# NeRF-3DTalker/NeRF-3DTalker-code

Measured on AMD Instinct MI355X. Metric: rendered frames/sec @512^2 x 64 samples/ray, higher is better.
Workload: dtype bf16; 1 GPU; cfg2-R: 16 heads/GPU/step, 64x64 rays x 64 samples -> fused MLP+composite -> neural renderer -> 512x512 RGB (+ background image); rays_per_frame=4096, samples_per_ray=64, parallelism=frames sharded over 1 rank(s), no data-path collective, ranks_seen_by_backend=1

## Files before the change

nerf-3dtalker-code_amd/csrc/nerf_aux.hip:

```cpp
#include "n3dt_device.h"
#include "n3dt_layout.h"
#include "n3dt_launch.h"

__device__ __forceinline__ float logical_weight(const N3dtMlpParams& p, int stage, int row, int col, int S, int A, int U) {
    const int in0 = N3DT_PE_DIM + S + U, in5 = N3DT_PE_DIM + S + N3DT_HID, inr = N3DT_HID + A;
    switch (stage) {
        case 0: return col < N3DT_PE_DIM ? p.weight[0][(size_t)row * in0 + col] : 0.0f;
        case 5:
            if (col < N3DT_PE_DIM) return p.weight[5][(size_t)row * in5 + col];
            if (col == N3DT_PE_DIM) return 0.0f;
            return p.weight[5][(size_t)row * in5 + N3DT_PE_DIM + S + (col - 64)];
        case 8: return row == 0 ? p.weight[8][col] : 0.0f;
        case 10: return p.weight[10][(size_t)row * inr + col];
        default: return p.weight[stage][(size_t)row * N3DT_HID + col];
    }
}

__global__ __launch_bounds__(256) void small_gemm_kernel(int M, int N, int K, const float* __restrict__ A, long sam, long sak,
                                                                 const float* __restrict__ Bm, long sbn, long sbk,
                                                                 float* __restrict__ C, long ldc, int accumulate) {
    __shared__ float As[32][33], Bs[32][33];
    const int t = threadIdx.x, tx = t & 15, ty = t >> 4;
    const int m0 = blockIdx.y * 32, n0 = blockIdx.x * 32;
    float acc[2][2] = {{0.f, 0.f}, {0.f, 0.f}};
// ... 190 lines not shown
    }
}

extern "C" void n3dt_launch_fold(const N3dtGeom* g, const N3dtMlpParams* p, const float* shape, const float* appea,
                                 const float* audio, float* fold, int merged_rgb, hipStream_t stream) {
    hipLaunchKernelGGL(fold_latents_kernel, dim3(g->batch, N3DT_NSTAGE, FOLD_ROWGROUPS), dim3(256), 0, stream, *p, g->shape_dim,
                       g->appea_dim, g->audio_dim, merged_rgb, shape, appea, audio, fold);
}

__global__ __launch_bounds__(256) void rayfold_kernel(int n_rays, long total, const float* __restrict__ fold, const float* __restrict__ ray_bias,
                                                      float* __restrict__ rayfold) {
    const long i = (long)blockIdx.x * blockDim.x + threadIdx.x;
    if (i >= total * 48) return;
    const long ray = i / 48;
    const int o = (int)(i % 48) * 4;
    const f32x4 f = *reinterpret_cast<const f32x4*>(fold + (size_t)(ray / n_rays) * N3DT_FOLD_STRIDE + n3dt_bias_offset(10) + o);
    const f32x4 r = *reinterpret_cast<const f32x4*>(ray_bias + (size_t)ray * N3DT_RAYFOLD_STRIDE + o);
    *reinterpret_cast<f32x4*>(rayfold + (size_t)ray * N3DT_RAYFOLD_STRIDE + o) = f32x4{f[0] + r[0], f[1] + r[1], f[2] + r[2], f[3] + r[3]};
}
extern "C" void n3dt_launch_rayfold(const N3dtGeom* g, const float* fold, const float* ray_bias, hipStream_t s) {
    const long total = (long)g->batch * g->n_rays;
    float* rayfold = const_cast<float*>(fold) + n3dt_rayfold_offset(g->batch);
    hipLaunchKernelGGL(rayfold_kernel, dim3((unsigned)((total * 48 + 255) / 256)), dim3(256), 0, s, g->n_rays, total, fold, ray_bias, rayfold);
}

__global__ __launch_bounds__(256) void ray_vd_bias_kernel(N3dtGeom g, const float* __restrict__ w_vd, long ld_w, const float* __restrict__ xy,
                                                          const float* __restrict__ R, const float* __restrict__ Kinv,
                                                          float* __restrict__ ray_bias) {
    __shared__ float wl[192 * 27];
    for (int i = threadIdx.x; i < 192 * 27; i += blockDim.x) wl[i] = w_vd[(size_t)(i / 27) * ld_w + i % 27];
    __syncthreads();
    const int lane = threadIdx.x & 63, wave = threadIdx.x >> 6;
    const long total = (long)g.batch * g.n_rays;
    for (long rayg = (long)blockIdx.x * 4 + wave; rayg < total; rayg += (long)gridDim.x * 4) {
        const int b = (int)(rayg / g.n_rays), ray = (int)(rayg % g.n_rays);
        const float x = xy[(int64_t)b * g.xy_stride_b + 0 * g.xy_stride_c + (int64_t)ray * g.xy_stride_r];
        const float y = xy[(int64_t)b * g.xy_stride_b + 1 * g.xy_stride_c + (int64_t)ray * g.xy_stride_r];
        float d[3], l;
        n3dt_ray_setup(R + b * 9, Kinv + b * 9, x, y, d, l);
        float pe[27];
        pe[0] = d[0]; pe[1] = d[1]; pe[2] = d[2];
#pragma unroll
        for (int k = 0; k < 4; ++k)
#pragma unroll
            for (int i = 0; i < 3; ++i) {
                const float a = d[i] * (float)(1 << k);
                pe[3 + 6 * k + i] = sinf(a);
                pe[3 + 6 * k + 3 + i] = cosf(a);
            }
#pragma unroll
        for (int u = 0; u < 3; ++u) {
            const int o = lane + 64 * u;
            float acc = 0.0f;
#pragma unroll
            for (int j = 0; j < 27; ++j) acc = fmaf(wl[o * 27 + j], pe[j], acc);
            ray_bias[(size_t)rayg * N3DT_RAYFOLD_STRIDE + o] = acc;
        }
    }
}
extern "C" void n3dt_launch_ray_vd_bias(const N3dtGeom* g, const float* w_vd, long ld_w, const float* xy, const float* R, const float* Kinv,
                                        float* ray_bias, hipStream_t s) {
    const long total = (long)g->batch * g->n_rays;
    long grid = (total + 3) / 4;
    if (grid > 2048) grid = 2048;
    hipLaunchKernelGGL(ray_vd_bias_kernel, dim3((unsigned)grid), dim3(256), 0, s, *g, w_vd, ld_w, xy, R, Kinv, ray_bias);
}

#define HEAD_RAYS 8
#define HEAD_MAX_BPR 64
__global__ __launch_bounds__(256) void ray_head_kernel(N3dtGeom g, int bpr, int bs, const float* __restrict__ part,
                                                       const float* __restrict__ wlocal, const float* __restrict__ tail,
                                                       const float* __restrict__ bg_featmap, int bg_hwc, float* __restrict__ fg_feat,
                                                       float* __restrict__ bg_alpha, float* __restrict__ depth,
                                                       float* __restrict__ weight, float* __restrict__ merge_feat,
                                                       float* __restrict__ rayrec) {
    __shared__ float G[HEAD_RAYS][N3DT_G];
    __shared__ float pref[HEAD_RAYS][HEAD_MAX_BPR];
    __shared__ float wsum_s[HEAD_RAYS], dsum_s[HEAD_RAYS];
    const long nrays_total = (long)g.batch * g.n_rays;
    const long ray0 = (long)blockIdx.x * HEAD_RAYS;
    const int t = threadIdx.x;
    if (t < HEAD_RAYS) {
        long rg = ray0 + t;
        float Trun = 1.0f, ws = 0.0f, ds = 0.0f;
        if (rg < nrays_total) {
            for (int k = 0; k < bpr; ++k) {
                const float* po = part + ((size_t)rg * bpr + k) * N3DT_PART_STRIDE + N3DT_G;
                pref[t][k] = Trun;
                ws += Trun * po[0];
                ds += Trun * po[1];
                Trun *= po[2];
            }
        }
        wsum_s[t] = ws;
        dsum_s[t] = ds;
    }
    __syncthreads();
    for (int i = t; i < HEAD_RAYS * N3DT_G; i += 256) {
        int r = i / N3DT_G, j = i % N3DT_G;
        long rg = ray0 + r;
        float acc = 0.0f;
        if (rg < nrays_total)
            for (int k = 0; k < bpr; ++k) acc += pref[r][k] * part[((size_t)rg * bpr + k) * N3DT_PART_STRIDE + j];
        G[r][j] = acc;
        if (rayrec && rg < nrays_total) rayrec[(size_t)rg * N3DT_PART_STRIDE + j] = acc;
    }
    __syncthreads();
    if (rayrec && t < HEAD_RAYS && ray0 + t < nrays_total) {
        float* rec = rayrec + (size_t)(ray0 + t) * N3DT_PART_STRIDE + N3DT_G;
        rec[0] = wsum_s[t];
        rec[1] = dsum_s[t];
        rec[2] = 0.0f;
        rec[3] = 0.0f;
    }
    const float* W2T = tail;
    const float b2 = tail[N3DT_G * N3DT_C + t];
    float acc[HEAD_RAYS];
#pragma unroll
    for (int r = 0; r < HEAD_RAYS; ++r) acc[r] = 0.0f;
    for (int j = 0; j < N3DT_G; ++j) {
        float wv = W2T[j * N3DT_C + t];
#pragma unroll
        for (int r = 0; r < HEAD_RAYS; ++r) acc[r] = fmaf(wv, G[r][j], acc[r]);
    }
#pragma unroll
    for (int r = 0; r < HEAD_RAYS; ++r) {
        long rg = ray0 + r;
        if (rg >= nrays_total) break;
        float fg = acc[r] + b2 * wsum_s[r];
        float ba = 1.0f - wsum_s[r];
        if (fg_feat) fg_feat[(size_t)rg * N3DT_C + t] = fg;
        if (merge_feat) {
            int ray = (int)(rg % g.n_rays);
            merge_feat[(size_t)rg * N3DT_C + t] = fg + ba * (bg_hwc ? bg_featmap[(size_t)ray * N3DT_C + t] : bg_featmap[(size_t)t * g.n_rays + ray]);
        }
        if (t == 0) {
            if (bg_alpha) bg_alpha[rg] = ba;
            if (depth) depth[rg] = dsum_s[r];
        }
    }
    if (weight) {
        for (int i = t; i < HEAD_RAYS * g.n_samples; i += 256) {
            int r = i / g.n_samples, s = i % g.n_samples;
            long rg = ray0 + r;
            if (rg < nrays_total) {
                int k = s / bs;
                weight[(size_t)rg * g.n_samples + s] = pref[r][k] * wlocal[((size_t)rg * bpr + k) * bs + (s % bs)];
            }
        }
    }
}

typedef __bf16 rh_bf16x8 __attribute__((ext_vector_type(8)));
#define RH_RAYS 32
template <bool MAP16, int PREC16 = N3DT_BF16>
__global__ __launch_bounds__(256, 4) void ray_head_mfma_kernel(N3dtGeom g, int bpr, int bs, const float* __restrict__ part,
                                                            const float* __restrict__ wlocal, const float* __restrict__ tail,
                                                            const float* __restrict__ bg_featmap, int bg_hwc,
                                                            float* __restrict__ fg_feat, float* __restrict__ bg_alpha,
                                                            float* __restrict__ depth, float* __restrict__ weight,
                                                            float* __restrict__ merge_feat, float* __restrict__ rayrec,
                                                            unsigned short* __restrict__ merge16, float* __restrict__ rgb0, const float* __restrict__ rgb_w,
                                                            const float* __restrict__ rgb_b) {
    __shared__ __attribute__((aligned(16))) float G[RH_RAYS][N3DT_G + 4];
    __shared__ float pref[RH_RAYS][HEAD_MAX_BPR];
    __shared__ float wsum_s[RH_RAYS], dsum_s[RH_RAYS];
    __shared__ float rgb_s[4][RH_RAYS][3];
    const long nrays_total = (long)g.batch * g.n_rays;
    const long ray0 = (long)blockIdx.x * RH_RAYS;
    const int t = threadIdx.x, lane = t & 63, wave = t >> 6;
    if (MAP16) rayrec = nullptr;
    if (t < RH_RAYS) {
        const long rg = ray0 + t;
        float Trun = 1.0f, ws = 0.0f, ds = 0.0f;
        if (rg < nrays_total) {
            for (int k = 0; k < bpr; ++k) {
                const float* po = part + ((size_t)rg * bpr + k) * N3DT_PART_STRIDE + N3DT_G;
                pref[t][k] = Trun;
                ws += Trun * po[0];
                ds += Trun * po[1];
                Trun *= po[2];
            }
        }
        wsum_s[t] = ws;
        dsum_s[t] = ds;
    }
    __syncthreads();
    static_assert(N3DT_G % 4 == 0 && (N3DT_PART_STRIDE * 4) % 16 == 0 && RH_RAYS * (N3DT_G / 4) % 256 == 0, "whole quads");
    constexpr int QPR = N3DT_G / 4, NQ = RH_RAYS * QPR / 256;
    if (bpr <= 2) {
        f32x4 v[NQ][2];
        float pf[NQ][2];
#pragma unroll
        for (int u = 0; u < NQ; ++u) {
            const int i = t + 256 * u, r = i / QPR, q = i % QPR;
            const long rg = min(ray0 + r, nrays_total - 1);
            const float* p0 = part + (size_t)rg * bpr * N3DT_PART_STRIDE + 4 * q;
            v[u][0] = *reinterpret_cast<const f32x4*>(p0);
            v[u][1] = *reinterpret_cast<const f32x4*>(p0 + (bpr == 2 ? N3DT_PART_STRIDE : 0));
            pf[u][0] = pref[r][0];
            pf[u][1] = bpr == 2 ? pref[r][1] : 0.0f;
        }
#pragma unroll
        for (int u = 0; u < NQ; ++u) {
            const int i = t + 256 * u, r = i / QPR, q = i % QPR;
            f32x4 a;
#pragma unroll
            for (int e = 0; e < 4; ++e) a[e] = pf[u][0] * v[u][0][e] + pf[u][1] * v[u][1][e];
            const bool in = ray0 + r < nrays_total;
            if (!in) a = f32x4{0.0f, 0.0f, 0.0f, 0.0f};
            *reinterpret_cast<f32x4*>(&G[r][4 * q]) = a;
            if (rayrec && in) *reinterpret_cast<f32x4*>(rayrec + (size_t)(ray0 + r) * N3DT_PART_STRIDE + 4 * q) = a;
        }
    } else {
        for (int i = t; i < RH_RAYS * N3DT_G; i += 256) {
            const int r = i / N3DT_G, j = i % N3DT_G;
            const long rg = ray0 + r;
            float acc = 0.0f;
            if (rg < nrays_total)
                for (int k = 0; k < bpr; ++k) acc += pref[r][k] * part[((size_t)rg * bpr + k) * N3DT_PART_STRIDE + j];
            G[r][j] = acc;
            if (rayrec && rg < nrays_total) rayrec[(size_t)rg * N3DT_PART_STRIDE + j] = acc;
        }
    }
    __syncthreads();
    if (rayrec && t < RH_RAYS && ray0 + t < nrays_total) {
        float* rec = rayrec + (size_t)(ray0 + t) * N3DT_PART_STRIDE + N3DT_G;
        rec[0] = wsum_s[t];
        rec[1] = dsum_s[t];
        rec[2] = 0.0f;
        rec[3] = 0.0f;
    }
    const int r31 = lane & 31, h = lane >> 5;
    f32x16 acc[2];
#pragma unroll
    for (int i = 0; i < 2; ++i)
#pragma unroll
        for (int r = 0; r < 16; ++r) acc[i][r] = 0.0f;
    const rh_bf16x8* w2frags = reinterpret_cast<const rh_bf16x8*>(tail + n3dt_tail_w2_frags_offset());
#pragma unroll 2
    for (int ks = 0; ks < N3DT_G / 16; ++ks) {
        const int k0 = 16 * ks + 8 * h;
        rh_bf16x8 a_hi, a_lo;
        const f32x4 g0 = *reinterpret_cast<const f32x4*>(&G[r31][k0]), g1 = *reinterpret_cast<const f32x4*>(&G[r31][k0 + 4]);
#pragma unroll
        for (int j = 0; j < 8; ++j) {
            const float v = j < 4 ? g0[j] : g1[j - 4];
            const __bf16 hi = (__bf16)v;
            a_hi[j] = hi;
            a_lo[j] = (__bf16)(v - (float)hi);
        }
#pragma unroll
        for (int i = 0; i < 2; ++i) {
            const rh_bf16x8* fr = w2frags + ((size_t)(ks * 8 + 2 * wave + i) * 2) * 64 + lane;
            const rh_bf16x8 b_hi = fr[0], b_lo = fr[64];
            acc[i] = __builtin_amdgcn_mfma_f32_32x32x16_bf16(a_hi, b_hi, acc[i], 0, 0, 0);
            acc[i] = __builtin_amdgcn_mfma_f32_32x32x16_bf16(a_hi, b_lo, acc[i], 0, 0, 0);
            acc[i] = __builtin_amdgcn_mfma_f32_32x32x16_bf16(a_lo, b_hi, acc[i], 0, 0, 0);
        }
    }
    float pr[MAP16 ? 16 : 1][3];
    if constexpr (!MAP16) {
#pragma unroll
        for (int i = 0; i < 2; ++i) {
            const int c = 64 * wave + 32 * i + r31;
            const float b2 = tail[N3DT_G * N3DT_C + c];
            float bgv[16];
#pragma unroll
            for (int r = 0; r < 16; ++r) {
                const int rr = (r & 3) + 8 * (r >> 2) + 4 * h;
                const long rg = min(ray0 + rr, nrays_total - 1);
                const int ray = (int)(rg % g.n_rays);
                bgv[r] = merge_feat ? (bg_hwc ? bg_featmap[(size_t)ray * N3DT_C + c] : bg_featmap[(size_t)c * g.n_rays + ray]) : 0.0f;
            }
#pragma unroll
            for (int r = 0; r < 16; ++r) {
                const int rr = (r & 3) + 8 * (r >> 2) + 4 * h;
                const long rg = ray0 + rr;
                if (rg >= nrays_total) continue;
                const float fg = acc[i][r] + b2 * wsum_s[rr];
                if (fg_feat) fg_feat[(size_t)rg * N3DT_C + c] = fg;
                if (merge_feat) merge_feat[(size_t)rg * N3DT_C + c] = fg + (1.0f - wsum_s[rr]) * bgv[r];
            }
        }
    } else {
#pragma unroll
        for (int i = 0; i < 2; ++i) {
            const int c = 64 * wave + 32 * i + r31;
            const float b2 = tail[N3DT_G * N3DT_C + c];
            float w3[3] = {0.0f, 0.0f, 0.0f};
            if (rgb0) {
#pragma unroll
                for (int k = 0; k < 3; ++k) w3[k] = rgb_w[k * N3DT_C + c];
            }
#pragma unroll
            for (int r0 = 0; r0 < 16; r0 += 8) {
                float bgv[8];
#pragma unroll
                for (int r = r0; r < r0 + 8; ++r) {
                    const int rr = (r & 3) + 8 * (r >> 2) + 4 * h;
                    const long rg = min(ray0 + rr, nrays_total - 1);
                    const int ray = (int)(rg % g.n_rays);
                    bgv[r - r0] = bg_featmap[(size_t)ray * N3DT_C + c];
                }
#pragma unroll
                for (int r = r0; r < r0 + 8; ++r) {
                    const int rr = (r & 3) + 8 * (r >> 2) + 4 * h;
                    const long rg = ray0 + rr;
                    const float mg = (acc[i][r] + b2 * wsum_s[rr]) + (1.0f - wsum_s[rr]) * bgv[r - r0];
#pragma unroll
                    for (int k = 0; k < 3; ++k) pr[MAP16 ? r : 0][k] = i == 0 ? w3[k] * mg : fmaf(w3[k], mg, pr[MAP16 ? r : 0][k]);
                    if (merge16 && rg < nrays_total)
                        merge16[(size_t)rg * N3DT_C + c] = PREC16 == N3DT_BF16 ? __builtin_bit_cast(unsigned short, (__bf16)mg)
                                                                               : __builtin_bit_cast(unsigned short, (_Float16)mg);
                }
                __builtin_amdgcn_sched_barrier(0);
            }
            __builtin_amdgcn_sched_barrier(0);
        }
    }
    if constexpr (MAP16) if (rgb0) {
#pragma unroll
        for (int step = 0; step < 4; ++step) {
            const int n = 8 >> step, off = 16 >> step;
            const bool up = (r31 & off) != 0;
#pragma unroll
            for (int r = 0; r < n; ++r)
#pragma unroll
                for (int k = 0; k < 3; ++k) {
                    const float keep = up ? pr[r + n][k] : pr[r][k], send = up ? pr[r][k] : pr[r + n][k];
                    pr[r][k] = keep + __shfl_xor(send, off, 64);
                }
        }
#pragma unroll
        for (int k = 0; k < 3; ++k) pr[0][k] += __shfl_xor(pr[0][k], 1, 64);
        if ((r31 & 1) == 0) {
            const int rsel = (r31 >> 1) & 15;
            const int rr = (rsel & 3) + 8 * (rsel >> 2) + 4 * h;
#pragma unroll
            for (int k = 0; k < 3; ++k) rgb_s[wave][rr][k] = pr[0][k];
        }
        __syncthreads();
        if (t < 3 * RH_RAYS) {
            const int rr = t % RH_RAYS, k = t / RH_RAYS;
            const long rg = ray0 + rr;
            if (rg < nrays_total) {
                const float v = (rgb_s[0][rr][k] + rgb_s[1][rr][k]) + (rgb_s[2][rr][k] + rgb_s[3][rr][k]) + rgb_b[k];
                const long img = rg / g.n_rays, p = rg % g.n_rays;
                rgb0[(size_t)(img * 3 + k) * g.n_rays + p] = v;
            }
        }
    }
    if (t < RH_RAYS && ray0 + t < nrays_total) {
        if (bg_alpha) bg_alpha[ray0 + t] = 1.0f - wsum_s[t];
        if (depth) depth[ray0 + t] = dsum_s[t];
    }
    if (weight) {
        for (int i = t; i < RH_RAYS * g.n_samples; i += 256) {
            const int r = i / g.n_samples, s = i % g.n_samples;
            const long rg = ray0 + r;
            if (rg < nrays_total) {
                const int k = s / bs;
                weight[(size_t)rg * g.n_samples + s] = pref[r][k] * wlocal[((size_t)rg * bpr + k) * bs + (s % bs)];
            }
        }
    }
}

extern "C" void n3dt_launch_ray_head_mfma(const N3dtGeom* g, int bpr, int bs, const float* part, const float* wlocal,
                                          const float* tail, const float* bg_featmap, int bg_hwc, float* fg_feat, float* bg_alpha,
                                          float* depth, float* weight, float* merge_feat, float* rayrec, hipStream_t stream) {
    const long nrays_total = (long)g->batch * g->n_rays;
    const int grid = (int)((nrays_total + RH_RAYS - 1) / RH_RAYS);
    hipLaunchKernelGGL(ray_head_mfma_kernel<false>, dim3(grid), dim3(256), 0, stream, *g, bpr, bs, part, wlocal, tail,
                       merge_feat ? bg_featmap : nullptr, bg_hwc, fg_feat, bg_alpha, depth, weight, merge_feat, rayrec,
                       (unsigned short*)nullptr, (float*)nullptr, (const float*)nullptr, (const float*)nullptr);
}

extern "C" void n3dt_launch_ray_head_mfma16(const N3dtGeom* g, int bpr, int bs, const float* part, const float* wlocal,
                                            const float* tail, const float* bg_featmap, int bg_hwc, float* fg_feat, float* bg_alpha,
                                            float* depth, float* weight, float* merge_feat, void* merge16, int prec16, float* rgb0,
                                            const float* rgb_w, const float* rgb_b, hipStream_t stream) {
    const long nrays_total = (long)g->batch * g->n_rays;
    const int grid = (int)((nrays_total + RH_RAYS - 1) / RH_RAYS);
    if (fg_feat || merge_feat) {
        hipLaunchKernelGGL(ray_head_mfma_kernel<false>, dim3(grid), dim3(256), 0, stream, *g, bpr, bs, part, wlocal, tail,
                           merge_feat ? bg_featmap : nullptr, bg_hwc, fg_feat, (float*)nullptr, (float*)nullptr, (float*)nullptr, merge_feat,
                           (float*)nullptr, (unsigned short*)nullptr, (float*)nullptr, (const float*)nullptr, (const float*)nullptr);
    }
    if (prec16 == N3DT_BF16)
        hipLaunchKernelGGL((ray_head_mfma_kernel<true, N3DT_BF16>), dim3(grid), dim3(256), 0, stream, *g, bpr, bs, part, wlocal, tail, bg_featmap,
                           bg_hwc, (float*)nullptr, bg_alpha, depth, weight, (float*)nullptr, (float*)nullptr,
                           reinterpret_cast<unsigned short*>(merge16), rgb0, rgb_w, rgb_b);
    else
        hipLaunchKernelGGL((ray_head_mfma_kernel<true, N3DT_F16>), dim3(grid), dim3(256), 0, stream, *g, bpr, bs, part, wlocal, tail, bg_featmap,
                           bg_hwc, (float*)nullptr, bg_alpha, depth, weight, (float*)nullptr, (float*)nullptr,
                           reinterpret_cast<unsigned short*>(merge16), rgb0, rgb_w, rgb_b);
}

extern "C" void n3dt_launch_ray_head(const N3dtGeom* g, int bpr, int bs, const float* part, const float* wlocal,
                                     const float* tail, const float* bg_featmap, int bg_hwc, float* fg_feat, float* bg_alpha,
                                     float* depth, float* weight, float* merge_feat, hipStream_t stream) {
    const long nrays_total = (long)g->batch * g->n_rays;
    const int grid = (int)((nrays_total + HEAD_RAYS - 1) / HEAD_RAYS);
    hipLaunchKernelGGL(ray_head_kernel, dim3(grid), dim3(256), 0, stream, *g, bpr, bs, part, wlocal, tail,
                       merge_feat ? bg_featmap : nullptr, bg_hwc, fg_feat, bg_alpha, depth, weight, merge_feat, (float*)nullptr);
}

// ... 127 lines not shown
```

nerf-3dtalker-code_amd/csrc/nr_blur_mfma.inc:

```
#define NBM_TR 4
#define NBM_TC 8
#define NBM_IMG 4096
#define NBM_BUF (NBM_IMG + 512)
#define NBM_WAVE (2 * NBM_BUF)

template <int N>
__device__ __forceinline__ void nbm_wait_vm() {
    asm volatile("s_waitcnt vmcnt(%0)" ::"i"(N) : "memory");
}

template <int PREC, bool NET>
__global__ __launch_bounds__(256) void blur_mfma_q_kernel(const int nb, const int H, const int W, const int K, const unsigned short* __restrict__ hid,
                                                          const float* __restrict__ bias, unsigned short* __restrict__ net,
                                                          const float* __restrict__ Wrgb, const float* __restrict__ brgb,
                                                          const float* __restrict__ rgb_lo, float* __restrict__ rgb_out, const int final_sigmoid,
                                                          float* __restrict__ rgb_out2, const int n_tiles) {
    typedef typename X16<PREC>::frag frag;
    extern __shared__ __attribute__((aligned(16))) unsigned char lds[];
    const int wave = __builtin_amdgcn_readfirstlane(threadIdx.x >> 6);
    const int lane = threadIdx.x & 63, c = lane & 31, hh = lane >> 5;
    const int nchunk = K >> 5;
    unsigned char* const wave_lds = lds + wave * NBM_WAVE;
    unsigned char* const a2_lds = lds + 4 * NBM_WAVE;
    float* const bias_lds = reinterpret_cast<float*>(a2_lds + (size_t)nchunk * 2 * 2 * 2 * 3 * 16);
// ... 136 lines not shown
    nimg = img; nR0 = R0; nC0 = C0;
    setup_tile(img, R0, C0);
    issue_item(0, 0);
    int younger = 0;
    float p0 = 0.0f, p1 = 0.0f;
    f32x16 acc2;
    for (;;) {
        const int R = R0 + (c >> 3), C = C0 + (c & 7);
        int nt = t, nc = chunk + 1;
        if (nc == nchunk) {
            nt = t + nw;
            nc = 0;
        }
        const bool has_next = nt < n_tiles;
        if (younger >= 5) nbm_wait_vm<5>();
        else if (younger >= 3) nbm_wait_vm<3>();
        else if (younger >= 2) nbm_wait_vm<2>();
        else nbm_wait_vm<0>();
        const unsigned img_addr = wave_addr + buf * NBM_BUF + tr_off;
        x16_u32x2 q0[4], q1[4];
        x16_tr_issue<0>(q0[0], img_addr);
        x16_tr_issue<256>(q1[0], img_addr);
        x16_tr_issue<1024>(q0[1], img_addr);
        x16_tr_issue<1280>(q1[1], img_addr);
        x16_tr_issue<2048>(q0[2], img_addr);
        x16_tr_issue<2304>(q1[2], img_addr);
        x16_tr_issue<3072>(q0[3], img_addr);
        x16_tr_issue<3328>(q1[3], img_addr);
        if (chunk == 0) {
#pragma unroll
            for (int r = 0; r < 16; ++r) acc2[r] = 0.0f;
            p0 = p1 = 0.0f;
            if (rgb_lo) {
                const float* win = reinterpret_cast<const float*>(wave_lds + buf * NBM_BUF + NBM_IMG) + ((R >> 1) - (R0 >> 1)) * 6 + ((C >> 1) - (C0 >> 1));
                float wr[3] = {wr_in[0], wr_in[1], wr_in[2]}, wc[3] = {wc_in[0], wc_in[1], wc_in[2]};
                if (R0 < 2 || R0 + NBM_TR > H2 - 2 || H < 3) n3dt_up_blur_w3(R, H, wr);
                if (C0 < 2 || C0 + NBM_TC > W2 - 2 || W < 3) n3dt_up_blur_w3(C, W, wc);
                const float* wa = win + (hh ? 48 : 0);
                float tmp[3] = {0.0f, 0.0f, 0.0f}, tm1[3] = {0.0f, 0.0f, 0.0f};
#pragma unroll
                for (int a = 0; a < 3; ++a)
#pragma unroll
                    for (int b = 0; b < 3; ++b) {
                        tmp[b] = fmaf(wr[a], wa[6 * a + b], tmp[b]);
                        tm1[b] = fmaf(wr[a], win[24 + 6 * a + b], tm1[b]);
                    }
#pragma unroll
                for (int b = 0; b < 3; ++b) {
                    p0 = fmaf(wc[b], tmp[b], p0);
                    p1 = fmaf(wc[b], tm1[b], p1);
                }
            }
        }
        const f32x4* bp = reinterpret_cast<const f32x4*>(bias_lds + chunk * 32 + hh * 16);
        const f32x4 bq0 = bp[0], bq1 = bp[1], bq2 = bp[2], bq3 = bp[3];
        x16_tr_settle();
#pragma unroll
        for (int s = 0; s < 4; ++s) asm volatile("" : "+v"(q0[s]), "+v"(q1[s]));
        if (has_next) {
            if (nc == 0) {
                where(nt, nimg, nR0, nC0);
                setup_tile(nimg, nR0, nC0);
            }
            issue_item(nc, buf ^ 1);
        }
        younger = 0;
        f32x16 acc;
#pragma unroll
        for (int r = 0; r < 16; ++r) acc[r] = 0.0f;
#pragma unroll
        for (int s = 0; s < 4; ++s) {
            const x16_u32x4 v = {q0[s][0], q0[s][1], q1[s][0], q1[s][1]};
            acc = X16<PREC>::mfma(__builtin_bit_cast(frag, v), S[s], acc);
        }
        const float bb[16] = {bq0[0], bq0[1], bq0[2], bq0[3], bq1[0], bq1[1], bq1[2], bq1[3],
                              bq2[0], bq2[1], bq2[2], bq2[3], bq3[0], bq3[1], bq3[2], bq3[3]};
        float v[16];
#pragma unroll
        for (int r = 0; r < 16; ++r) {
            const float a = fmaf(acc[r], 0.0625f, bb[r]);
            v[r] = fmaxf(a, 0.2f * a);
        }
        const frag f0 = X16<PREC>::pack(v), f1 = X16<PREC>::pack(v + 8);
        if (NET) {
            unsigned char* const tb = wave_lds + buf * NBM_BUF;
            const x16_u32x4 w0 = __builtin_bit_cast(x16_u32x4, f0), w1 = __builtin_bit_cast(x16_u32x4, f1);
            unsigned char* const wrow = tb + c * 72 + 8 * hh;
            *reinterpret_cast<x16_u32x2*>(wrow) = x16_u32x2{w0[0], w0[1]};
            *reinterpret_cast<x16_u32x2*>(wrow + 16) = x16_u32x2{w0[2], w0[3]};
            *reinterpret_cast<x16_u32x2*>(wrow + 32) = x16_u32x2{w1[0], w1[1]};
            *reinterpret_cast<x16_u32x2*>(wrow + 48) = x16_u32x2{w1[2], w1[3]};
            __builtin_amdgcn_fence(__ATOMIC_RELEASE, "wavefront");
            __builtin_amdgcn_wave_barrier();
            __builtin_amdgcn_fence(__ATOMIC_ACQUIRE, "wavefront");
            unsigned char* const nbase = reinterpret_cast<unsigned char*>(net) + ((((size_t)img * H2 + R0) * W2 + C0) * K + chunk * 32) * 2;
#pragma unroll
            for (int jj = 0; jj < 2; ++jj) {
                const unsigned char* rrow = tb + ((lane >> 2) + 16 * jj) * 72 + 16 * (lane & 3);
                const x16_u32x2 lo = *reinterpret_cast<const x16_u32x2*>(rrow), hi = *reinterpret_cast<const x16_u32x2*>(rrow + 8);
                *reinterpret_cast<x16_u32x4*>(nbase + soff[jj]) = x16_u32x4{lo[0], lo[1], hi[0], hi[1]};
            }
            younger += 2;
        }
        {
            const unsigned char* ap = a2_lds + (size_t)(((chunk * 2) * 2 * 2 + hh) * 3 + (c < 3 ? c : 0)) * 16;
            const frag z = __builtin_bit_cast(frag, x16_u32x4{0u, 0u, 0u, 0u});
            const frag t0h = *reinterpret_cast<const frag*>(ap), t0l = *reinterpret_cast<const frag*>(ap + 6 * 16);
            const frag t1h = *reinterpret_cast<const frag*>(ap + 12 * 16), t1l = *reinterpret_cast<const frag*>(ap + 18 * 16);
            const bool live = c < 3;
            acc2 = X16<PREC>::mfma(live ? t0l : z, f0, acc2);
            acc2 = X16<PREC>::mfma(live ? t1l : z, f1, acc2);
            acc2 = X16<PREC>::mfma(live ? t0h : z, f0, acc2);
            acc2 = X16<PREC>::mfma(live ? t1h : z, f1, acc2);
        }
        if (nc == 0) {
            const float p2 = __shfl(p0, c + 32, 64);
            if (!hh) {
                float r0 = acc2[0] + b0 + p0, r1 = acc2[1] + b1 + p1, r2 = acc2[2] + b2 + p2;
                if (final_sigmoid) {
                    r0 = 1.0f / (1.0f + __expf(-r0));
                    r1 = 1.0f / (1.0f + __expf(-r1));
                    r2 = 1.0f / (1.0f + __expf(-r2));
                }
                const size_t o = (size_t)img * 3 * HW2 + (size_t)R * W2 + C;
                rgb_out[o] = r0;
                rgb_out[o + HW2] = r1;
                rgb_out[o + 2 * HW2] = r2;
                if (rgb_out2) {
                    rgb_out2[o] = r0;
                    rgb_out2[o + HW2] = r1;
                    rgb_out2[o + 2 * HW2] = r2;
                }
            }
            younger += 3;
        }
        if (!has_next) break;
        t = nt;
        chunk = nc;
        buf ^= 1;
        img = nimg;
        R0 = nR0;
        C0 = nC0;
    }
}

#define NBM8_SLOTS 112
#define NBM8_IMG (NBM8_SLOTS * 64)
#define NBM8_BUF (NBM8_IMG + 512)
#ifndef NBM8_DB
#define NBM8_DB 0
#endif
#define NBM8_WAVE ((NBM8_DB ? 2 : 1) * NBM8_BUF)

template <int PREC>
__global__ __launch_bounds__(256) void blur_mfma_last_kernel(const int nb, const int H, const int W, const unsigned short* __restrict__ hid,
                                                             const float* __restrict__ bias, const float* __restrict__ Wrgb,
                                                             const float* __restrict__ brgb, const float* __restrict__ rgb_lo,
                                                             float* __restrict__ rgb_out, const int final_sigmoid, float* __restrict__ rgb_out2,
                                                             const int n_tiles) {
    typedef typename X16<PREC>::frag frag;
    constexpr int K = 32;
    extern __shared__ __attribute__((aligned(16))) unsigned char lds[];
    const int wave = __builtin_amdgcn_readfirstlane(threadIdx.x >> 6);
    const int lane = threadIdx.x & 63, c = lane & 31, hh = lane >> 5;
    unsigned char* const wave_lds = lds + wave * NBM8_WAVE;
    unsigned char* const a2_lds = lds + 4 * NBM8_WAVE;
    float* const bias_lds = reinterpret_cast<float*>(a2_lds + 2 * 2 * 2 * 3 * 16);

    for (int i = threadIdx.x; i < 2 * 2 * 3; i += blockDim.x) {
        const int row = i % 3, half = (i / 3) & 1, s = i / 6;
        float w[8], rem[8];
#pragma unroll
        for (int e = 0; e < 8; ++e) {
            const int r = 8 * s + e, ch = (r & 3) + 8 * (r >> 2) + 4 * half;
            w[e] = Wrgb[(size_t)row * K + ch];
        }
        const frag hi = X16<PREC>::pack(w);
#pragma unroll
        for (int e = 0; e < 8; ++e) rem[e] = w[e] - (float)hi[e];
        const frag lo = X16<PREC>::pack(rem);
        *reinterpret_cast<frag*>(a2_lds + (size_t)((((s * 2 + 0) * 2 + half) * 3 + row) * 16)) = hi;
        *reinterpret_cast<frag*>(a2_lds + (size_t)((((s * 2 + 1) * 2 + half) * 3 + row) * 16)) = lo;
    }
    for (int i = threadIdx.x; i < 32; i += blockDim.x) {
        const int half = i >> 4, r = i & 15;
        bias_lds[i] = bias[(r & 3) + 8 * (r >> 2) + 4 * half];
    }
    asm volatile("s_waitcnt vmcnt(0)" ::: "memory");
    __syncthreads();

    frag S[4];
    {
        const int orow = c >> 3, ocol = c & 7;
#pragma unroll
        for (int s = 0; s < 4; ++s) {
            float w[8];
#pragma unroll
            for (int e = 0; e < 8; ++e) {
                const int k = 16 * s + 8 * hh + e, hr = k / 10, hc = k - 10 * hr;
                const int dr = hr - orow, dc = hc - ocol;
                const float wr = (k < 60 && dr >= 0 && dr <= 2) ? (dr == 1 ? 2.0f : 1.0f) : 0.0f;
                const float wc = (dc >= 0 && dc <= 2) ? (dc == 1 ? 2.0f : 1.0f) : 0.0f;
                w[e] = wr * wc;
            }
            S[s] = X16<PREC>::pack(w);
        }
    }
    const bool live = c < 3;
    const frag z = __builtin_bit_cast(frag, x16_u32x4{0u, 0u, 0u, 0u});
    frag t0h, t0l, t1h, t1l;
    {
        const unsigned char* ap = a2_lds + (size_t)((hh * 3 + (live ? c : 0)) * 16);
        t0h = *reinterpret_cast<const frag*>(ap);
        t0l = *reinterpret_cast<const frag*>(ap + 6 * 16);
        t1h = *reinterpret_cast<const frag*>(ap + 12 * 16);
        t1l = *reinterpret_cast<const frag*>(ap + 18 * 16);
        if (!live) t0h = t0l = t1h = t1l = z;
    }
    const int H2 = 2 * H, W2 = 2 * W;
    const size_t Mq = (size_t)nb * H * W;
    int ioff[7];
#pragma unroll
    for (int i = 0; i < 7; ++i) {
        int k = 16 * i + (lane >> 2);
        if (k > 99) k = 99;
        const int hr = k / 10, hc = k - 10 * hr;
        const int q = 2 * ((hr + 1) & 1) + ((hc + 1) & 1);
        const long dR = (hr - 1) >> 1, dC = (hc - 1) >> 1;
        ioff[i] = (int)((((long)q * (long)Mq + dR * W + dC) * K + 8 * (lane & 3)) * 2);
    }
    int pch[2], prow[2], pcol[2];
#pragma unroll
    for (int i = 0; i < 2; ++i) {
        int j = 64 * i + lane;
        if (j > 107) j = 107;
        pch[i] = j / 36;
        prow[i] = (j - 36 * pch[i]) / 6;
        pcol[i] = j - 36 * pch[i] - 6 * prow[i];
    }
    const unsigned img_addr = (unsigned)(size_t)(LDS_AS unsigned char*)wave_lds + x16_tr_lane_offset_natural(lane);
    const int tiles_x = W2 / 8, tiles_y = H2 / 8, per_img = tiles_x * tiles_y;
    const int tx_shift = (tiles_x & (tiles_x - 1)) == 0 ? 31 - __builtin_clz(tiles_x) : -1;
    const int ty_shift = (tiles_y & (tiles_y - 1)) == 0 ? 31 - __builtin_clz(tiles_y) : -1;
    const bool pow2 = tx_shift >= 0 && ty_shift >= 0;
    auto where = [&](const int t, int& img, int& R0, int& C0) {
        if (pow2) {
            C0 = (t & (tiles_x - 1)) * 8;
            R0 = ((t >> tx_shift) & (tiles_y - 1)) * 8;
            img = t >> (tx_shift + ty_shift);
        } else {
            img = t / per_img;
            const int tt = t - img * per_img, ty = tt / tiles_x;
            R0 = ty * 8;
            C0 = (tt - ty * tiles_x) * 8;
        }
    };
    const bool r_ev = ((c >> 3) & 1) == 0, c_ev = (c & 1) == 0;
    const float wr_in[3] = {r_ev ? 0.3125f : 0.0625f, 0.625f, r_ev ? 0.0625f : 0.3125f};
    const float wc_in[3] = {c_ev ? 0.3125f : 0.0625f, 0.625f, c_ev ? 0.0625f : 0.3125f};
    const size_t HW2 = (size_t)H2 * W2;
    const float b0 = brgb[0], b1 = brgb[1], b2 = brgb[2];
    const int nw = gridDim.x * 4;

    auto issue_item = [&](const int img, const int R0, const int C0, const int buf) {
        unsigned char* const dstb = wave_lds + buf * NBM8_BUF;
        if (rgb_lo) {
#pragma unroll
            for (int i = 0; i < 2; ++i) {
                const int hr = min(max((R0 >> 1) - 1 + prow[i], 0), H - 1), wc = min(max((C0 >> 1) - 1 + pcol[i], 0), W - 1);
                const float* ps = rgb_lo + (((size_t)img * 3 + pch[i]) * H + hr) * W + wc;
                __builtin_amdgcn_global_load_lds((const GLOBAL_AS void*)ps, (LDS_AS void*)(dstb + NBM8_IMG + 256 * i), 4, 0, 0);
            }
        }
        const bool interior = R0 > 0 && R0 + 8 < H2 && C0 > 0 && C0 + 8 < W2;
        if (interior) {
            const unsigned char* base = reinterpret_cast<const unsigned char*>(hid) + (((size_t)img * H + (R0 >> 1)) * W + (C0 >> 1)) * K * 2;
#pragma unroll
            for (int i = 0; i < 7; ++i)
                __builtin_amdgcn_global_load_lds((const GLOBAL_AS void*)(base + ioff[i]), (LDS_AS void*)(dstb + i * 1024), 16, 0, 0);
        } else {
#pragma unroll
            for (int i = 0; i < 7; ++i) {
                int k = 16 * i + (lane >> 2);
                if (k > 99) k = 99;
                const int hr = k / 10, hc = k - 10 * hr;
                const int R = hreflect1(R0 - 1 + hr, H2), C = hreflect1(C0 - 1 + hc, W2);
                const int q = 2 * (R & 1) + (C & 1);
                const unsigned char* sp = reinterpret_cast<const unsigned char*>(hid) +
                                          (((size_t)q * Mq + ((size_t)img * H + (R >> 1)) * W + (C >> 1)) * K + 8 * (lane & 3)) * 2;
                __builtin_amdgcn_global_load_lds((const GLOBAL_AS void*)sp, (LDS_AS void*)(dstb + i * 1024), 16, 0, 0);
            }
        }
    };

    int t = blockIdx.x * 4 + wave;
    if (t >= n_tiles) return;
    int img, R0, C0;
    where(t, img, R0, C0);
    issue_item(img, R0, C0, 0);
    bool first = true;
    int buf = 0;
    for (;;) {
        const int nt = t + nw;
        const bool has_next = nt < n_tiles;
        if (first) nbm_wait_vm<0>();
        else nbm_wait_vm<NBM8_DB ? 6 : 3>();
        first = false;
        int nimg = img, nR0 = R0, nC0 = C0;
        if (NBM8_DB && has_next) {
            where(nt, nimg, nR0, nC0);
            issue_item(nimg, nR0, nC0, buf ^ 1);
        }
        const unsigned cur_addr = img_addr + buf * NBM8_BUF;
        float p0[2] = {0.0f, 0.0f}, p1[2] = {0.0f, 0.0f};
        if (rgb_lo) {
            const float* win0 = reinterpret_cast<const float*>(wave_lds + buf * NBM8_BUF + NBM8_IMG);
            const bool edge_c = C0 == 0 || C0 + 8 == W2 || W < 3;
#pragma unroll
            for (int j = 0; j < 2; ++j) {
                const int R = R0 + 4 * j + (c >> 3), C = C0 + (c & 7);
                float wr[3] = {wr_in[0], wr_in[1], wr_in[2]}, wc[3] = {wc_in[0], wc_in[1], wc_in[2]};
                if ((j == 0 && R0 == 0) || (j == 1 && R0 + 8 == H2) || H < 3) n3dt_up_blur_w3(R, H, wr);
                if (edge_c) n3dt_up_blur_w3(C, W, wc);
                const float* win = win0 + ((R >> 1) - (R0 >> 1)) * 6 + ((C >> 1) - (C0 >> 1));
                const float* wa = win + (hh ? 72 : 0);
                float tmp[3] = {0.0f, 0.0f, 0.0f}, tm1[3] = {0.0f, 0.0f, 0.0f};
#pragma unroll
                for (int a = 0; a < 3; ++a)
#pragma unroll
                    for (int b = 0; b < 3; ++b) {
                        tmp[b] = fmaf(wr[a], wa[6 * a + b], tmp[b]);
                        tm1[b] = fmaf(wr[a], win[36 + 6 * a + b], tm1[b]);
                    }
#pragma unroll
                for (int b = 0; b < 3; ++b) {
                    p0[j] = fmaf(wc[b], tmp[b], p0[j]);
                    p1[j] = fmaf(wc[b], tm1[b], p1[j]);
                }
            }
        }
#pragma unroll
        for (int j = 0; j < 2; ++j) {
            x16_u32x2 q0[4], q1[4];
            if (j == 0) {
                x16_tr_issue<0>(q0[0], cur_addr);
                x16_tr_issue<256>(q1[0], cur_addr);
                x16_tr_issue<1024>(q0[1], cur_addr);
                x16_tr_issue<1280>(q1[1], cur_addr);
                x16_tr_issue<2048>(q0[2], cur_addr);
                x16_tr_issue<2304>(q1[2], cur_addr);
                x16_tr_issue<3072>(q0[3], cur_addr);
                x16_tr_issue<3328>(q1[3], cur_addr);
            } else {
                x16_tr_issue<2560 + 0>(q0[0], cur_addr);
                x16_tr_issue<2560 + 256>(q1[0], cur_addr);
                x16_tr_issue<2560 + 1024>(q0[1], cur_addr);
                x16_tr_issue<2560 + 1280>(q1[1], cur_addr);
                x16_tr_issue<2560 + 2048>(q0[2], cur_addr);
                x16_tr_issue<2560 + 2304>(q1[2], cur_addr);
                x16_tr_issue<2560 + 3072>(q0[3], cur_addr);
                x16_tr_issue<2560 + 3328>(q1[3], cur_addr);
            }
            x16_tr_settle();
#pragma unroll
            for (int s = 0; s < 4; ++s) asm volatile("" : "+v"(q0[s]), "+v"(q1[s]));
            if (!NBM8_DB && j == 1 && has_next) {
                where(nt, nimg, nR0, nC0);
                issue_item(nimg, nR0, nC0, 0);
            }
            f32x16 acc;
#pragma unroll
            for (int r = 0; r < 16; ++r) acc[r] = 0.0f;
#pragma unroll
            for (int s = 0; s < 4; ++s) {
                const x16_u32x4 v = {q0[s][0], q0[s][1], q1[s][0], q1[s][1]};
                acc = X16<PREC>::mfma(__builtin_bit_cast(frag, v), S[s], acc);
            }
            float v[16];
            {
                const f32x4* bp = reinterpret_cast<const f32x4*>(bias_lds + hh * 16);
                const f32x4 bq0 = bp[0], bq1 = bp[1], bq2 = bp[2], bq3 = bp[3];
                const float bb[16] = {bq0[0], bq0[1], bq0[2], bq0[3], bq1[0], bq1[1], bq1[2], bq1[3],
                                      bq2[0], bq2[1], bq2[2], bq2[3], bq3[0], bq3[1], bq3[2], bq3[3]};
#pragma unroll
                for (int r = 0; r < 16; ++r) {
                    const float a = fmaf(acc[r], 0.0625f, bb[r]);
                    v[r] = fmaxf(a, 0.2f * a);
                }
            }
            const frag f0 = X16<PREC>::pack(v), f1 = X16<PREC>::pack(v + 8);
            f32x16 acc2;
#pragma unroll
            for (int r = 0; r < 16; ++r) acc2[r] = 0.0f;
            acc2 = X16<PREC>::mfma(t0l, f0, acc2);
            acc2 = X16<PREC>::mfma(t1l, f1, acc2);
            acc2 = X16<PREC>::mfma(t0h, f0, acc2);
            acc2 = X16<PREC>::mfma(t1h, f1, acc2);
            const float p2 = __shfl(p0[j], c + 32, 64);
            if (!hh) {
                const int R = R0 + 4 * j + (c >> 3), C = C0 + (c & 7);
                float r0 = acc2[0] + b0 + p0[j], r1 = acc2[1] + b1 + p1[j], r2 = acc2[2] + b2 + p2;
                if (final_sigmoid) {
                    r0 = 1.0f / (1.0f + __expf(-r0));
                    r1 = 1.0f / (1.0f + __expf(-r1));
                    r2 = 1.0f / (1.0f + __expf(-r2));
                }
                const size_t o = (size_t)img * 3 * HW2 + (size_t)R * W2 + C;
                rgb_out[o] = r0;
                rgb_out[o + HW2] = r1;
                rgb_out[o + 2 * HW2] = r2;
                if (rgb_out2) {
                    rgb_out2[o] = r0;
                    rgb_out2[o + HW2] = r1;
                    rgb_out2[o + 2 * HW2] = r2;
                }
            }
        }
        if (!has_next) break;
        t = nt;
        img = nimg;
        R0 = nR0;
        C0 = nC0;
        if (NBM8_DB) buf ^= 1;
    }
}

static inline bool nbm_supported(int nb, int H, int W, int K) {
    const char* e = getenv("N3DT_NR_BLUR_MFMA");
    if (e && atoi(e) == 0) return false;
    if (H < 2 || W < 4 || (H & 1) || (W & 3) || (K & 31) || K > 256) return false;
    return (size_t)4 * nb * H * W * K * 2 < ((size_t)1 << 31);
}

template <int PREC>
static void launch_blur_q(int nb, int H, int W, int K, const unsigned short* hid, const float* bias, unsigned short* net, const float* Wrgb,
                          const float* brgb, const float* rgb_lo, float* rgb_out, int final_sigmoid, float* rgb_out2, hipStream_t s) {
    if (!net && K == 32 && !(H & 3) && nbm_supported(nb, H, W, K) && !(getenv("N3DT_NR_BLUR_TILE8") && atoi(getenv("N3DT_NR_BLUR_TILE8")) == 0)) {
        const int n_tiles = nb * (2 * H / 8) * (2 * W / 8);
        const size_t lds_bytes = 4 * NBM8_WAVE + 2 * 2 * 2 * 3 * 16 + 32 * sizeof(float);
        auto kern = blur_mfma_last_kernel<PREC>;
        static int cus8 = 0, occ8 = 0;
        if (cus8 == 0) {
            int dev = 0, n = 0;
            (void)hipGetDevice(&dev);
            (void)hipDeviceGetAttribute(&n, hipDeviceAttributeMultiprocessorCount, dev);
            cus8 = n > 0 ? n : 256;
        }
        if (occ8 == 0 && (hipOccupancyMaxActiveBlocksPerMultiprocessor(&occ8, reinterpret_cast<const void*>(kern), 256, lds_bytes) != hipSuccess || occ8 < 1))
            occ8 = 2;
        int wgs = (n_tiles + 3) / 4;
        if (wgs > cus8 * occ8) wgs = cus8 * occ8;
        hipLaunchKernelGGL(kern, dim3((unsigned)wgs), dim3(256), lds_bytes, s, nb, H, W, hid, bias, Wrgb, brgb, rgb_lo, rgb_out, final_sigmoid, rgb_out2,
                           n_tiles);
        return;
    }
    if (nbm_supported(nb, H, W, K)) {
        const int n_tiles = nb * (2 * H / NBM_TR) * (2 * W / NBM_TC);
// ... 25 lines not shown
```

Before: 2244 frames/s.

## Pre-split ray-head G into bf16 hi/lo in LDS, prefetch weight frags, chunk blur tile walk

The ray-head kernel now splits the composited features into bf16 hi/lo pairs once, when writing them to shared memory. This replaces the per-k-step fp32 LDS reads and conversions inside the MFMA loop. The MFMA weight fragments are loaded through a triple-buffered register prefetch two steps ahead, and the part loads are hoisted before the transmittance prefix sync, so global latency overlaps other work. The blur kernel's tile walk groups blocks into eight contiguous spans, which likely changes locality across XCDs. Register pressure rises from the fragment buffers and full unrolling, and this may reduce occupancy under launch bounds (256,4).

```diff
diff --git a/nerf-3dtalker-code_amd/csrc/nerf_aux.hip b/nerf-3dtalker-code_amd/csrc/nerf_aux.hip
--- a/nerf-3dtalker-code_amd/csrc/nerf_aux.hip
+++ b/nerf-3dtalker-code_amd/csrc/nerf_aux.hip
@@ -366,6 +366,7 @@
 }
 
 typedef __bf16 rh_bf16x8 __attribute__((ext_vector_type(8)));
+typedef __bf16 rh_bf16x4 __attribute__((ext_vector_type(4)));
 #define RH_RAYS 32
 template <bool MAP16, int PREC16 = N3DT_BF16>
 __global__ __launch_bounds__(256, 4) void ray_head_mfma_kernel(N3dtGeom g, int bpr, int bs, const float* __restrict__ part,
@@ -376,7 +377,16 @@
                                                             float* __restrict__ merge_feat, float* __restrict__ rayrec,
                                                             unsigned short* __restrict__ merge16, float* __restrict__ rgb0, const float* __restrict__ rgb_w,
                                                             const float* __restrict__ rgb_b) {
-    __shared__ __attribute__((aligned(16))) float G[RH_RAYS][N3DT_G + 4];
+    constexpr int G_ROW = 4 * (N3DT_G + 4);
+    __shared__ __attribute__((aligned(16))) unsigned char Gs[RH_RAYS][G_ROW];
+    auto split4 = [](const f32x4 a, rh_bf16x4& hi, rh_bf16x4& lo) {
+#pragma unroll
+        for (int e = 0; e < 4; ++e) {
+            const __bf16 hv = (__bf16)a[e];
+            hi[e] = hv;
+            lo[e] = (__bf16)(a[e] - (float)hv);
+        }
+    };
     __shared__ float pref[RH_RAYS][HEAD_MAX_BPR];
     __shared__ float wsum_s[RH_RAYS], dsum_s[RH_RAYS];
     __shared__ float rgb_s[4][RH_RAYS][3];
@@ -384,6 +394,31 @@
     const long ray0 = (long)blockIdx.x * RH_RAYS;
     const int t = threadIdx.x, lane = t & 63, wave = t >> 6;
     if (MAP16) rayrec = nullptr;
+    const rh_bf16x8* w2frags = reinterpret_cast<const rh_bf16x8*>(tail + n3dt_tail_w2_frags_offset());
+    rh_bf16x8 bfr[3][4];
+    auto load_frags = [&](const int ks, rh_bf16x8(&b)[4]) {
+#pragma unroll
+        for (int i = 0; i < 2; ++i) {
+            const rh_bf16x8* fr = w2frags + ((size_t)(ks * 8 + 2 * wave + i) * 2) * 64 + lane;
+            b[2 * i] = fr[0];
+            b[2 * i + 1] = fr[64];
+        }
+    };
+    load_frags(0, bfr[0]);
+    load_frags(1, bfr[1]);
+    static_assert(N3DT_G % 4 == 0 && (N3DT_PART_STRIDE * 4) % 16 == 0 && RH_RAYS * (N3DT_G / 4) % 256 == 0, "whole quads");
+    constexpr int QPR = N3DT_G / 4, NQ = RH_RAYS * QPR / 256;
+    f32x4 v[NQ][2];
+    if (bpr <= 2) {
+#pragma unroll
+        for (int u = 0; u < NQ; ++u) {
+            const int i = t + 256 * u, r = i / QPR, q = i % QPR;
+            const long rg = min(ray0 + r, nrays_total - 1);
+            const float* p0 = part + (size_t)rg * bpr * N3DT_PART_STRIDE + 4 * q;
+            v[u][0] = *reinterpret_cast<const f32x4*>(p0);
+            v[u][1] = *reinterpret_cast<const f32x4*>(p0 + (bpr == 2 ? N3DT_PART_STRIDE : 0));
+        }
+    }
     if (t < RH_RAYS) {
         const long rg = ray0 + t;
         float Trun = 1.0f, ws = 0.0f, ds = 0.0f;
@@ -400,18 +435,11 @@
         dsum_s[t] = ds;
     }
     __syncthreads();
-    static_assert(N3DT_G % 4 == 0 && (N3DT_PART_STRIDE * 4) % 16 == 0 && RH_RAYS * (N3DT_G / 4) % 256 == 0, "whole quads");
-    constexpr int QPR = N3DT_G / 4, NQ = RH_RAYS * QPR / 256;
     if (bpr <= 2) {
-        f32x4 v[NQ][2];
         float pf[NQ][2];
 #pragma unroll
         for (int u = 0; u < NQ; ++u) {
-            const int i = t + 256 * u, r = i / QPR, q = i % QPR;
-            const long rg = min(ray0 + r, nrays_total - 1);
-            const float* p0 = part + (size_t)rg * bpr * N3DT_PART_STRIDE + 4 * q;
-            v[u][0] = *reinterpret_cast<const f32x4*>(p0);
-            v[u][1] = *reinterpret_cast<const f32x4*>(p0 + (bpr == 2 ? N3DT_PART_STRIDE : 0));
+            const int r = (t + 256 * u) / QPR;
             pf[u][0] = pref[r][0];
             pf[u][1] = bpr == 2 ? pref[r][1] : 0.0f;
         }
@@ -423,7 +451,11 @@
             for (int e = 0; e < 4; ++e) a[e] = pf[u][0] * v[u][0][e] + pf[u][1] * v[u][1][e];
             const bool in = ray0 + r < nrays_total;
             if (!in) a = f32x4{0.0f, 0.0f, 0.0f, 0.0f};
-            *reinterpret_cast<f32x4*>(&G[r][4 * q]) = a;
+            rh_bf16x4 hi, lo;
+            split4(a, hi, lo);
+            unsigned char* gp = &Gs[r][32 * (q >> 1) + 8 * (q & 1)];
+            *reinterpret_cast<rh_bf16x4*>(gp) = hi;
+            *reinterpret_cast<rh_bf16x4*>(gp + 16) = lo;
             if (rayrec && in) *reinterpret_cast<f32x4*>(rayrec + (size_t)(ray0 + r) * N3DT_PART_STRIDE + 4 * q) = a;
         }
     } else {
@@ -433,7 +465,10 @@
             float acc = 0.0f;
             if (rg < nrays_total)
                 for (int k = 0; k < bpr; ++k) acc += pref[r][k] * part[((size_t)rg * bpr + k) * N3DT_PART_STRIDE + j];
-            G[r][j] = acc;
+            const __bf16 hv = (__bf16)acc;
+            unsigned char* gp = &Gs[r][32 * (j >> 3) + 2 * (j & 7)];
+            *reinterpret_cast<__bf16*>(gp) = hv;
+            *reinterpret_cast<__bf16*>(gp + 16) = (__bf16)(acc - (float)hv);
             if (rayrec && rg < nrays_total) rayrec[(size_t)rg * N3DT_PART_STRIDE + j] = acc;
         }
     }
@@ -451,23 +486,15 @@
     for (int i = 0; i < 2; ++i)
 #pragma unroll
         for (int r = 0; r < 16; ++r) acc[i][r] = 0.0f;
-    const rh_bf16x8* w2frags = reinterpret_cast<const rh_bf16x8*>(tail + n3dt_tail_w2_frags_offset());
-#pragma unroll 2
+#pragma unroll
     for (int ks = 0; ks < N3DT_G / 16; ++ks) {
-        const int k0 = 16 * ks + 8 * h;
-        rh_bf16x8 a_hi, a_lo;
-        const f32x4 g0 = *reinterpret_cast<const f32x4*>(&G[r31][k0]), g1 = *reinterpret_cast<const f32x4*>(&G[r31][k0 + 4]);
-#pragma unroll
-        for (int j = 0; j < 8; ++j) {
-            const float v = j < 4 ? g0[j] : g1[j - 4];
-            const __bf16 hi = (__bf16)v;
-            a_hi[j] = hi;
-            a_lo[j] = (__bf16)(v - (float)hi);
-        }
+        if (ks + 2 < N3DT_G / 16) load_frags(ks + 2, bfr[(ks + 2) % 3]);
+        __builtin_amdgcn_sched_barrier(0);
+        const unsigned char* gp = &Gs[r31][32 * (2 * ks + h)];
+        const rh_bf16x8 a_hi = *reinterpret_cast<const rh_bf16x8*>(gp), a_lo = *reinterpret_cast<const rh_bf16x8*>(gp + 16);
 #pragma unroll
         for (int i = 0; i < 2; ++i) {
-            const rh_bf16x8* fr = w2frags + ((size_t)(ks * 8 + 2 * wave + i) * 2) * 64 + lane;
-            const rh_bf16x8 b_hi = fr[0], b_lo = fr[64];
+            const rh_bf16x8 b_hi = bfr[ks % 3][2 * i], b_lo = bfr[ks % 3][2 * i + 1];
             acc[i] = __builtin_amdgcn_mfma_f32_32x32x16_bf16(a_hi, b_hi, acc[i], 0, 0, 0);
             acc[i] = __builtin_amdgcn_mfma_f32_32x32x16_bf16(a_hi, b_lo, acc[i], 0, 0, 0);
             acc[i] = __builtin_amdgcn_mfma_f32_32x32x16_bf16(a_lo, b_hi, acc[i], 0, 0, 0);
diff --git a/nerf-3dtalker-code_amd/csrc/nr_blur_mfma.inc b/nerf-3dtalker-code_amd/csrc/nr_blur_mfma.inc
--- a/nerf-3dtalker-code_amd/csrc/nr_blur_mfma.inc
+++ b/nerf-3dtalker-code_amd/csrc/nr_blur_mfma.inc
@@ -312,6 +312,18 @@
 #endif
 #define NBM8_WAVE ((NBM8_DB ? 2 : 1) * NBM8_BUF)
 
+struct NbmWalk {
+    int first, end, step;
+};
+__device__ __forceinline__ NbmWalk nbm_walk(const int wave, const int n_tiles) {
+    const int g = blockIdx.x, G = gridDim.x;
+    if ((G & 7) == 0 && (n_tiles & 7) == 0) {
+        const int span = n_tiles >> 3, x = g & 7;
+        return NbmWalk{x * span + (g >> 3) * 4 + wave, (x + 1) * span, G >> 1};
+    }
+    return NbmWalk{g * 4 + wave, n_tiles, G * 4};
+}
+
 template <int PREC>
 __global__ __launch_bounds__(256) void blur_mfma_last_kernel(const int nb, const int H, const int W, const unsigned short* __restrict__ hid,
                                                              const float* __restrict__ bias, const float* __restrict__ Wrgb,
@@ -420,7 +432,8 @@
     const float wc_in[3] = {c_ev ? 0.3125f : 0.0625f, 0.625f, c_ev ? 0.0625f : 0.3125f};
     const size_t HW2 = (size_t)H2 * W2;
     const float b0 = brgb[0], b1 = brgb[1], b2 = brgb[2];
-    const int nw = gridDim.x * 4;
+    const NbmWalk walk = nbm_walk(wave, n_tiles);
+    const int nw = walk.step;
 
     auto issue_item = [&](const int img, const int R0, const int C0, const int buf) {
         unsigned char* const dstb = wave_lds + buf * NBM8_BUF;
@@ -453,8 +466,8 @@
         }
     };
 
-    int t = blockIdx.x * 4 + wave;
-    if (t >= n_tiles) return;
+    int t = walk.first;
+    if (t >= walk.end) return;
     int img, R0, C0;
     where(t, img, R0, C0);
     issue_item(img, R0, C0, 0);
@@ -462,7 +475,7 @@
     int buf = 0;
     for (;;) {
         const int nt = t + nw;
-        const bool has_next = nt < n_tiles;
+        const bool has_next = nt < walk.end;
         if (first) nbm_wait_vm<0>();
         else nbm_wait_vm<NBM8_DB ? 6 : 3>();
         first = false;
```

After: 2246 frames/s, median of 6. No clear change (+0.1%).
